# soedinglab/spacedust

Measured on AMD Instinct MI355X. Metric: clustersearch throughput (genome-pairs/s; SW GCUPS alongside), higher is better.
Workload: dtype int16

## Files before the change

### spacedust_amd/csrc/hip/sd_sw.hip

```cpp
#include "sd_common.h"
#include <unistd.h>


#include <algorithm>
#include <cmath>
#include <cstring>
#include <memory>
#include <omp.h>
#include <numeric>

#include "../host/sd_host.h"
#include "sd_sw_pk.h"

namespace {

using sdpk::SwTask;

template <int RT>
__global__ void __launch_bounds__(64)
sw_score_kernel(const SwTask *__restrict__ tasks, uint32_t nTasks, const uint8_t *__restrict__ qRes,
                const int8_t *__restrict__ qBias, const uint8_t *__restrict__ tRes, const int8_t *__restrict__ mat,
                int go, int ge, int32_t *__restrict__ out, uint2 *__restrict__ boundary,
                const uint32_t *__restrict__ order ,
                const int8_t *__restrict__ qProf ) {
// ... 611 lines not shown
            int x = ii - band;
            x = x > 0 ? x : 0;
            x = jj - x;
            ok = ok && x >= 0 && x < width_d;
            bool same = false;
            if (ok) {
                const int byte = dirs[(size_t) 16 * ii + (x >> 1)];
                const int code = (x & 1) ? (byte >> 4) : (byte & 15);
                ok = (code & 12) == 0;
                same = sq[ii] == st[jj];
            }
            const uint32_t okMask = (uint32_t) (__ballot(ok) >> sh);
            const uint32_t sameMask = (uint32_t) (__ballot(same) >> sh);
            const int run = okMask == 0xFFFFFFFFu ? 32 : __builtin_ctz(~okMask);
            const uint32_t runMask = run == 32 ? 0xFFFFFFFFu : ((1u << run) - 1u);
            if (l < run) o[-1 - l] = 'M';
            ids += __builtin_popcount(sameMask & runMask);
            i -= run;
            j -= run;
            o -= run;
            len += run;
        }
        if (going && (i > 0 || j > 0)) {
            if (i < 0 || j < 0) bad = true;
            int x = i - band;
            x = x > 0 ? x : 0;
            x = j - x;
            if (x < 0 || x >= width_d) bad = true;
            if (!bad) {
                const int byte = dirs[(size_t) 16 * i + (x >> 1)];
                const int code = (x & 1) ? (byte >> 4) : (byte & 15);
                int dcode;
                const int dE = (code & 1) ? 3 : 2, dF = (code & 2) ? 5 : 4;
                if (state == 0) dcode = dE;
                else if (state == 1) dcode = dF;
                else dcode = (code & 4) ? dE : ((code & 8) ? dF : 1);
                char c;
                switch (dcode) {
                    case 1: ids += (sq[i] == st[j]); --i; --j; state = 2; c = 'M'; break;
                    case 2: --i; state = 0; c = 'I'; break;
                    case 3: --i; state = 2; c = 'I'; break;
                    case 4: --j; state = 1; c = 'D'; break;
                    default: --j; state = 2; c = 'D'; break;
                }
                --o;
                if (l == 0) *o = c;
                len++;
            }
        }
        going = going && !bad && (i > 0 || j > 0);
    }
    if (!have || !reached || l != 0) return;
    if (bad || i != 0 || j != 0) {
        res[2 * id] = -1;
        return;
    }
    ids += (sq[0] == st[0]);
    *--o = 'M';
    len++;
    res[2 * id] = len;
    res[2 * id + 1] = ids;
}

template <int RT, int LW, bool MULTI, bool WIDE, bool SHARED>
void launchScorePk(sd_ctx *ctx, const SwTask *dTasks, const uint32_t *dOrder, uint32_t n, const sd_seqset *q,
                   const sd_seqset *t, const int8_t *dMat, int go, int ge, int32_t *dOut, uint2 *dBound) {
    if (n == 0) return;
    constexpr uint32_t perWave = 2 * (64 / LW);
    dim3 grid((n + perWave - 1) / perWave), block(64);
    hipLaunchKernelGGL((sdpk::sw_score_pk_kernel<RT, LW, MULTI, WIDE, SHARED>), grid, block, 0, ctx->stream, dTasks, n, q->dRes, q->dBias,
                       t->dRes, dMat, go, ge, dOut, dBound, dOrder, (const int8_t *) q->dProf);
}

template <int RT, bool SHARED>
void launchScorePkAligned(sd_ctx *ctx, const SwTask *dTasks, const uint32_t *dOrder, uint32_t n, const sd_seqset *q, const sd_seqset *t,
                          const int8_t *dMat, int go, int ge, int32_t *dOut) {
    if (n == 0) return;
    constexpr uint32_t perWave = 4;
    dim3 grid((n + perWave - 1) / perWave), block(64);
    hipLaunchKernelGGL((sdpk::sw_score_pk_aligned_kernel<RT, SHARED>), grid, block, 0, ctx->stream, dTasks, n, q->dRes, q->dBias, t->dRes,
                       dMat, go, ge, dOut, dOrder, (const int8_t *) q->dProf);
}

int rtClass(int n) {
    if (n <= 128) return 4;
    if (n <= 256) return 8;
    if (n <= 512) return 16;
    return 32;
}

template <int RT>
void launchScore(sd_ctx *ctx, const SwTask *dTasks, uint32_t n, const sd_seqset *q, const sd_seqset *t,
                 const int8_t *dMat, int go, int ge, int32_t *dOut, uint2 *dBound) {
    if (n == 0) return;
    dim3 grid((n + 1) / 2), block(64);
    hipLaunchKernelGGL(sw_score_kernel<RT>, grid, block, 0, ctx->stream, dTasks, n, q->dRes, q->dBias, t->dRes, dMat,
                       go, ge, dOut, dBound, (const uint32_t *) nullptr, (const int8_t *) q->dProf);
}

template <int RT>
void launchScoreIdx(sd_ctx *ctx, const SwTask *dTasks, const uint32_t *dOrder, uint32_t n, const sd_seqset *q,
                    const sd_seqset *t, const int8_t *dMat, int go, int ge, int32_t *dOut, uint2 *dBound) {
    if (n == 0) return;
    dim3 grid((n + 1) / 2), block(64);
    hipLaunchKernelGGL(sw_score_kernel<RT>, grid, block, 0, ctx->stream, dTasks, n, q->dRes, q->dBias, t->dRes, dMat,
                       go, ge, dOut, dBound, dOrder, (const int8_t *) q->dProf);
}

int runScoreTasks(sd_ctx *ctx, std::vector<SwTask> &tasks, const sd_seqset *q, const sd_seqset *t, const int8_t *dMat,
                  int go, int ge, std::vector<int32_t> &hOut, uint32_t nSlots, uint64_t *cells, const char *tag = "a") {
    hOut.assign((size_t) nSlots * 3, 0);
    if (tasks.empty()) return SD_OK;
    HostScope hsAll(ctx, "score.total");
    const size_t n = tasks.size();
    constexpr int NB = 4 * 1024;
    auto keyOf = [](const SwTask &t) {
        const int c = rtClass(t.n);
        const int ci = c == 4 ? 0 : (c == 8 ? 1 : (c == 16 ? 2 : 3));
        return (uint32_t) ci * 1024u + (uint32_t) (1023 - std::min(t.tL >> 4, 1023));
    };
    SwTask *sorted = nullptr;
    SD_HIP(ctx, pinGet(ctx, (std::string("sw.tasks.") + tag).c_str(), n, &sorted));
    uint64_t boundTotal = 0, cellSum = 0;
    size_t classBegin[5] = {0, 0, 0, 0, 0};
    {
        int T = 1;
#pragma omp parallel
        {
#pragma omp single
            T = omp_get_num_threads();
        }
        T = std::max(1, std::min(T, 64));
        std::vector<uint32_t> hist((size_t) T * NB, 0);
#pragma omp parallel num_threads(T) reduction(+ : cellSum)
        {
            const int th = omp_get_thread_num();
            const size_t lo = n * th / T, hi = n * (th + 1) / T;
            uint32_t *hh = &hist[(size_t) th * NB];
            for (size_t i = lo; i < hi; i++) {
                hh[keyOf(tasks[i])]++;
                cellSum += (uint64_t) tasks[i].n * (uint64_t) tasks[i].tL;
            }
        }
        uint64_t run = 0;
        for (int bkt = 0; bkt < NB; bkt++) {
            if ((bkt & 1023) == 0) classBegin[bkt >> 10] = run;
            for (int th = 0; th < T; th++) {
                const uint32_t c = hist[(size_t) th * NB + bkt];
                hist[(size_t) th * NB + bkt] = (uint32_t) run;
                run += c;
            }
        }
        classBegin[4] = run;
#pragma omp parallel num_threads(T)
        {
            const int th = omp_get_thread_num();
            const size_t lo = n * th / T, hi = n * (th + 1) / T;
            uint32_t *hh = &hist[(size_t) th * NB];
            for (size_t i = lo; i < hi; i++) sorted[hh[keyOf(tasks[i])]++] = tasks[i];
        }
    }
    *cells += cellSum;
    for (size_t i = classBegin[3]; i < classBegin[4]; i++) {
        if (sorted[i].n > 1024) {
            sorted[i].boundOff = boundTotal;
            boundTotal += (uint64_t) sorted[i].tL;
        }
    }
    SwTask *dTasks = nullptr;
    int32_t *dOut = nullptr;
    uint2 *dBound = nullptr;
    int32_t *hPin = nullptr;
    SD_HIP(ctx, wsGet(ctx, "sw.tasks", n, &dTasks));
    SD_HIP(ctx, wsGet(ctx, "sw.out", (size_t) nSlots * 3, &dOut));
    SD_HIP(ctx, wsGet(ctx, "sw.bound", std::max<uint64_t>(boundTotal, 1), &dBound));
    SD_HIP(ctx, pinGet(ctx, "sw.hout", (size_t) nSlots * 3, &hPin));
    SD_HIP(ctx, hipMemcpyAsync(dTasks, sorted, n * sizeof(SwTask), hipMemcpyHostToDevice, ctx->stream));
    SD_HIP(ctx, hipMemsetAsync(dOut, 0, (size_t) nSlots * 3 * sizeof(int32_t), ctx->stream));
    static const int classes[4] = {4, 8, 16, 32};
    for (int ci = 0; ci < 4; ci++) {
        const size_t begin = classBegin[ci], end = classBegin[ci + 1];
        if (end == begin) continue;
        const uint32_t cnt = (uint32_t) (end - begin);
        {
            ProfScope ps(ctx, "sw_score");
            switch (classes[ci]) {
                case 4: launchScore<4>(ctx, dTasks + begin, cnt, q, t, dMat, go, ge, dOut, dBound); break;
                case 8: launchScore<8>(ctx, dTasks + begin, cnt, q, t, dMat, go, ge, dOut, dBound); break;
                case 16: launchScore<16>(ctx, dTasks + begin, cnt, q, t, dMat, go, ge, dOut, dBound); break;
                default: launchScore<32>(ctx, dTasks + begin, cnt, q, t, dMat, go, ge, dOut, dBound); break;
            }
        }
        SD_HIP(ctx, hipGetLastError());
    }
    SD_HIP(ctx, hipMemcpyAsync(hPin, dOut, (size_t) nSlots * 3 * sizeof(int32_t), hipMemcpyDeviceToHost, ctx->stream));
    SD_HIP(ctx, sdStreamSync(ctx));
    memcpy(hOut.data(), hPin, (size_t) nSlots * 3 * sizeof(int32_t));
    return SD_OK;
}


constexpr uint32_t N_NARROW_CLASSES = 24;
constexpr uint32_t FIRST_NARROW_MULTI = 21;
constexpr uint32_t N_PK_CLASSES = 14;
constexpr uint32_t FIRST_MULTI_PK = 11;
constexpr uint32_t FIRST_WIDE_CLASS = N_NARROW_CLASSES;
constexpr uint32_t FIRST_INT32_CLASS = FIRST_WIDE_CLASS + N_PK_CLASSES;
constexpr uint32_t N_SCORE_CLASSES = FIRST_INT32_CLASS + 4;
static_assert(N_SCORE_CLASSES < 63, "class boundaries are found by one 64-lane wavefront; six class bits in the pair key");
enum ScoreKernel { SCORE_PK = 0, SCORE_PK_WIDE = 1, SCORE_INT32 = 2 };
constexpr uint32_t KEY_INVALID = N_SCORE_CLASSES * 1024u;
__host__ __device__ __forceinline__ bool scoreClassIsMulti(uint32_t ci) {
    return (ci >= FIRST_NARROW_MULTI && ci < FIRST_WIDE_CLASS) || (ci >= FIRST_WIDE_CLASS + FIRST_MULTI_PK && ci < FIRST_INT32_CLASS);
}
__device__ __forceinline__ uint32_t scoreKey(int n, int tL, int kernel, int wideRowLimit = 800) {
    int ci;
    if (kernel == SCORE_PK_WIDE && min(n, tL) > wideRowLimit) kernel = SCORE_INT32;
    if (kernel == SCORE_INT32 || tL > 65535) {
        ci = FIRST_INT32_CLASS + (n <= 128 ? 0 : (n <= 256 ? 1 : (n <= 512 ? 2 : 3)));
    } else if (kernel == SCORE_PK_WIDE) {
        if (n <= 192) ci = n <= 128 ? 0 : 1;
        else if (n <= 384) ci = 2 + (n - 193) / 32;
        else if (n <= 768) ci = n <= 512 ? 8 : (n <= 640 ? 9 : 10);
        else ci = min((int) FIRST_MULTI_PK + (n + 511) / 512 - 2, 13);
        ci += FIRST_WIDE_CLASS;
    } else {
        if (n <= 128) ci = 0;
        else if (n <= 768) ci = (n + 31) / 32 - 4;
        else ci = min((int) FIRST_NARROW_MULTI + (n + 511) / 512 - 2, (int) FIRST_WIDE_CLASS - 1);
    }
    return (uint32_t) ci * 1024u + (uint32_t) (1023 - min(tL >> 4, 1023));
}

struct DevGateParams {
    int go, ge, matMin, swMode, covMode, wideRowLimit;
    float covThr;
    double evalThr;
    double lambda, K, aI, bI, alphaI, betaI, aJ, bJ, alphaJ, betaJ, sigma, tau, viThr, vjThr, cThr, dbResidues;
};

__device__ double devEvalue(const DevGateParams &e, double y_, double qLen) {
    const double m_ = e.dbResidues, n_ = qLen;
    const double const_val = 0.3989422804014327;
    double tmp = e.aI * y_ + e.bI;
    double m_li_y = m_ - tmp;
    double vi_y = fmax(e.viThr, e.alphaI * y_ + e.betaI);
    double sqrt_vi_y = sqrt(vi_y);
    double m_F = sqrt_vi_y == 0.0 ? 1e100 : m_li_y / sqrt_vi_y;
    double P_m_F = 0.5 * erfc(-sqrt(0.5) * m_F);
    double E_m_F = -const_val * exp(-0.5 * m_F * m_F);
    double p1 = m_li_y * P_m_F - sqrt_vi_y * E_m_F;
    tmp = e.aJ * y_ + e.bJ;
    double n_lj_y = n_ - tmp;
    double vj_y = fmax(e.vjThr, e.alphaJ * y_ + e.betaJ);
    double sqrt_vj_y = sqrt(vj_y);
    double n_F = sqrt_vj_y == 0.0 ? 1e100 : n_lj_y / sqrt_vj_y;
    double P_n_F = 0.5 * erfc(-sqrt(0.5) * n_F);
    double E_n_F = -const_val * exp(-0.5 * n_F * n_F);
    double p2 = n_lj_y * P_n_F - sqrt_vj_y * E_n_F;
    double c_y = fmax(e.cThr, e.sigma * y_ + e.tau);
    double area = p1 * p2 + c_y * (P_m_F * P_n_F);
    return e.K * exp(-e.lambda * y_) * area;
}

__device__ __forceinline__ float devCov(unsigned int startPos, unsigned int endPos, unsigned int len) {
    return (min(len, max(startPos, endPos)) - min(startPos, endPos) + 1) / (float) len;
}
__device__ __forceinline__ bool devHasCoverage(float covThr, int covMode, float qCov, float tCov) {
    switch (covMode) {
        case 0: return (qCov >= covThr) && (tCov >= covThr);
        case 2: return qCov >= covThr;
        case 1: return tCov >= covThr;
        default: return true;
    }
}

__global__ void __launch_bounds__(256)
k_pre_word(uint32_t nPairs, const uint32_t *__restrict__ pairQ, const uint32_t *__restrict__ pairT, const uint16_t *__restrict__ pairDiag,
           const uint32_t *__restrict__ fwdKeys, const uint64_t *__restrict__ qOff, const uint64_t *__restrict__ tOff,
           const uint8_t *__restrict__ qRes, const int8_t *__restrict__ qBias, const uint8_t *__restrict__ tRes, const int8_t *__restrict__ mat,
           const int8_t *__restrict__ qProf, const int32_t *__restrict__ minBias, int matMin, uint8_t *__restrict__ preWord,
           uint32_t *__restrict__ pass1Keys) {
    __shared__ int8_t smat[441];
    for (int x = threadIdx.x; x < 441; x += blockDim.x) smat[x] = mat[x];
    __syncthreads();
    const uint32_t i = blockIdx.x * blockDim.x + threadIdx.x;
    if (i >= nPairs) return;
    uint8_t pw = 0;
    const uint32_t key = fwdKeys[i];
    if (key != KEY_INVALID) {
        const uint64_t qo = qOff[pairQ[i]], to = tOff[pairT[i]];
        const int qL = (int) (qOff[pairQ[i] + 1] - qo), tL = (int) (tOff[pairT[i] + 1] - to);
        if (qL < 32768 && tL < 32768 && pairDiag[i] != 0x8000) {
            const int d = (int) (int16_t) pairDiag[i];
            int q0 = d >= 0 ? d : 0, t0 = d >= 0 ? 0 : -d;
            const int n = min(qL - q0, tL - t0);
            const int need = 255 - (abs(matMin) + abs(minBias[pairQ[i]]));
            int run = 0, best = 0;
            for (int x = 0; x < n && best < need; x++) {
                const int qr = qRes[qo + q0 + x], tr = tRes[to + t0 + x];
                run += qProf ? (int) qProf[(qo + q0 + x) * 21 + tr] : (int) smat[tr * 21 + qr] + (int) qBias[qo + q0 + x];
                run = run < 0 ? 0 : run;
                best = run > best ? run : best;
            }
            pw = best >= need ? 1 : 0;
        }
    }
// ... 357 lines not shown
    if (!keep) {
        res[i].btLen = 0;
        btLen[i] = 0;
    }
}

__global__ void __launch_bounds__(256)
k_accept(uint32_t nPairs, const sd_sw_result *__restrict__ res, const uint8_t *__restrict__ ident, uint8_t *__restrict__ acc) {
    const uint32_t i = blockIdx.x * blockDim.x + threadIdx.x;
    if (i >= nPairs) return;
    const sd_sw_result &r = res[i];
    acc[i] = (ident[i] || (r.btLen > 0 && r.qStart >= 0 && r.tStart >= 0)) ? 1 : 0;
}
__global__ void __launch_bounds__(256)
k_accept_compact(uint32_t nPairs, const sd_sw_result *__restrict__ res, const uint8_t *__restrict__ acc,
                 const uint64_t *__restrict__ pos, sd_sw_result *__restrict__ outRes, uint32_t *__restrict__ outIdx) {
    const uint32_t i = blockIdx.x * blockDim.x + threadIdx.x;
    if (i >= nPairs || !acc[i]) return;
    outRes[pos[i]] = res[i];
    outIdx[pos[i]] = i;
}
#include "sd_scan_sort.h"

template <typename T>
int devExclusiveScan(sd_ctx *ctx, const T *in, uint64_t *out, size_t n) {
    uint64_t *tmp = nullptr;
    SD_HIP(ctx, wsGet(ctx, "al.scantmp", sdScanTmpBytes(n) / sizeof(uint64_t) + 32, &tmp));
    SD_HIP(ctx, (sdScanLaunch<T, ScanSum64, false, uint64_t>(ctx->stream, in, out, n, tmp)));
    return SD_OK;
}
int devInclusiveMax(sd_ctx *ctx, const uint32_t *in, uint32_t *out, size_t n) {
    uint32_t *tmp = nullptr;
    SD_HIP(ctx, wsGet(ctx, "al.scantmp32", sdScanTmpBytes(n) / sizeof(uint32_t) + 32, &tmp));
    SD_HIP(ctx, (sdScanLaunch<uint32_t, ScanMax32, true, uint32_t>(ctx->stream, in, out, n, tmp)));
    return SD_OK;
}

int devSortPairs(sd_ctx *ctx, const uint32_t *kIn, uint32_t *kOut, const uint32_t *vIn, uint32_t *vOut, size_t n, int endBit) {
    if (n == 0) return SD_OK;
    uint32_t *kTmp = nullptr, *vTmp = nullptr, *cnt = nullptr;
    SD_HIP(ctx, wsGet(ctx, "al.sortK", n, &kTmp));
    SD_HIP(ctx, wsGet(ctx, "al.sortV", n, &vTmp));
    SD_HIP(ctx, wsGet(ctx, "al.sortCounts", sdRadixSortCountsBytes() / sizeof(uint32_t), &cnt));
    SD_HIP(ctx, sdRadixSortPairs(ctx->stream, kIn, vIn, kOut, vOut, kTmp, vTmp, (uint32_t) n, 0, endBit, cnt));
    return SD_OK;
}

__global__ void __launch_bounds__(256)
k_bound_need(uint32_t nPairs, const SwTask *__restrict__ tasks, const uint32_t *__restrict__ keys, uint64_t *__restrict__ need) {
    const uint32_t i = blockIdx.x * blockDim.x + threadIdx.x;
    if (i >= nPairs) return;
    uint64_t v = 0;
    if (keys[i] != KEY_INVALID) {
        const uint32_t ci = keys[i] >> 10;
        if (scoreClassIsMulti(ci)) v = 2ull * (uint64_t) tasks[i].tL;
        else if (ci == N_SCORE_CLASSES - 1 && tasks[i].n > 1024) v = (uint64_t) tasks[i].tL;
    }
    need[i] = v;
}
__global__ void __launch_bounds__(256)
k_bound_apply(uint32_t nPairs, SwTask *__restrict__ tasks, const uint64_t *__restrict__ off) {
    const uint32_t i = blockIdx.x * blockDim.x + threadIdx.x;
    if (i >= nPairs) return;
    tasks[i].boundOff = off[i];
}

constexpr uint32_t PAIR_NONE = 0xFFFFFFFFu;
constexpr int PAIR_QUERY_BITS = 17;
__global__ void __launch_bounds__(256)
k_pair_keys(uint32_t n, const uint32_t *__restrict__ keys, const uint32_t *__restrict__ pairQ, uint32_t *__restrict__ key2) {
    const uint32_t i = blockIdx.x * blockDim.x + threadIdx.x;
    if (i >= n) return;
    const uint32_t k = keys[i];
    key2[i] = k == KEY_INVALID ? 0xFFFFFFFFu : ((k >> 10) << 26) | (pairQ[i] << 9) | ((k & 1023u) >> 1);
}
__global__ void __launch_bounds__(256)
k_pair_heads(uint32_t n, const uint32_t *__restrict__ keyS, uint32_t *__restrict__ headPos) {
    const uint32_t p = blockIdx.x * blockDim.x + threadIdx.x;
    if (p >= n) return;
    const bool head = p == 0 || (keyS[p] >> 9) != (keyS[p - 1] >> 9);
    headPos[p] = head ? p : 0u;
}
__global__ void __launch_bounds__(256)
k_pair_leaders(uint32_t n, const uint32_t *__restrict__ keyS, const uint32_t *__restrict__ runStart, uint8_t *__restrict__ leader) {
    const uint32_t p = blockIdx.x * blockDim.x + threadIdx.x;
    if (p > n) return;
    uint8_t v = 0;
    if (p < n && (keyS[p] >> 26) < FIRST_INT32_CLASS) {
        const uint32_t o = p - runStart[p];
        v = (o & 1u) == 0 ? 1 : 0;
        const bool lastOfRun = p + 1 >= n || (keyS[p + 1] >> 9) != (keyS[p] >> 9);
        const uint32_t pairs = (o + 1 + 1) / 2;
        if (lastOfRun) v += (uint8_t) (pairs & 1u);
    }
    leader[p] = v;
}
__global__ void __launch_bounds__(256)
k_pair_emit(uint32_t n, const uint32_t *__restrict__ keyS, const uint32_t *__restrict__ vals, const uint32_t *__restrict__ runStartOf,
            const uint64_t *__restrict__ pairIdx, uint32_t *__restrict__ order2) {
    const uint32_t p = blockIdx.x * blockDim.x + threadIdx.x;
    if (p >= n || (keyS[p] >> 26) >= FIRST_INT32_CLASS || ((p - runStartOf[p]) & 1u)) return;
    const uint64_t w = pairIdx[p];
    order2[2 * w] = vals[p];
    const bool mate = p + 1 < n && (keyS[p + 1] >> 9) == (keyS[p] >> 9);
    order2[2 * w + 1] = mate ? vals[p + 1] : PAIR_NONE;
}
__global__ void k_pair_bounds(const uint32_t *__restrict__ keyS, uint32_t n, const uint64_t *__restrict__ pairIdx,
                              uint32_t *__restrict__ b, int nb) {
    const int c = threadIdx.x;
    if (c >= nb) return;
    const uint32_t want = (uint32_t) c << 26;
    uint32_t lo = 0, hi = n;
    while (lo < hi) {
        const uint32_t mid = (lo + hi) >> 1;
        if (keyS[mid] < want) lo = mid + 1;
        else hi = mid;
    }
    b[c] = (uint32_t) pairIdx[lo];
}

int devRunScore(sd_ctx *ctx, uint32_t nPairs, const uint32_t *dKeys, const uint32_t *dVals, uint32_t *dKeysSorted,
                uint32_t *dOrder, uint32_t *dBounds, SwTask *dTasks, uint64_t *dScanA, uint64_t *dScanB,
                const sd_seqset *q, const sd_seqset *t, const int8_t *dMat, int go, int ge, int32_t *dOut,
                uint32_t *nValid, const uint32_t *dPairQ ) {
    const unsigned grid = (nPairs + 255) / 256;
    int rc = SD_OK;
    uint32_t *dOrder2 = nullptr, *dPairBounds = nullptr;
    if (dPairQ) {
        uint32_t *dKey2 = nullptr, *dVals2 = nullptr, *dHead = nullptr, *dRunStart = nullptr;
        uint64_t *dPairIdx = nullptr;
        uint8_t *dLeader = nullptr;
        SD_HIP(ctx, wsGet(ctx, "sp.key2", (size_t) nPairs, &dKey2));
        SD_HIP(ctx, wsGet(ctx, "sp.vals2", (size_t) nPairs, &dVals2));
        SD_HIP(ctx, wsGet(ctx, "sp.head", (size_t) nPairs, &dHead));
        SD_HIP(ctx, wsGet(ctx, "sp.runstart", (size_t) nPairs, &dRunStart));
        SD_HIP(ctx, wsGet(ctx, "sp.leader", (size_t) nPairs + 1, &dLeader));
        SD_HIP(ctx, wsGet(ctx, "sp.pairidx", (size_t) nPairs + 1, &dPairIdx));
        const size_t order2Cap = (size_t) 4 * nPairs + 8;
        SD_HIP(ctx, wsGet(ctx, "sp.order2", order2Cap, &dOrder2));
        SD_HIP(ctx, hipMemsetAsync(dOrder2, 0xFF, order2Cap * sizeof(uint32_t), ctx->stream));
        SD_HIP(ctx, wsGet(ctx, "sp.bounds", 64, &dPairBounds));
        hipLaunchKernelGGL(k_pair_keys, dim3(grid), dim3(256), 0, ctx->stream, nPairs, dKeys, dPairQ, dKey2);
        rc = devSortPairs(ctx, dKey2, dKeysSorted, dVals, dVals2, nPairs, 32);
        if (rc != SD_OK) return rc;
        dOrder = dVals2;
        hipLaunchKernelGGL(k_pair_heads, dim3(grid), dim3(256), 0, ctx->stream, nPairs, dKeysSorted, dHead);
        rc = devInclusiveMax(ctx, dHead, dRunStart, nPairs);
        if (rc != SD_OK) return rc;
        hipLaunchKernelGGL(k_pair_leaders, dim3((nPairs + 256) / 256), dim3(256), 0, ctx->stream, nPairs, dKeysSorted, dRunStart, dLeader);
        rc = devExclusiveScan(ctx, (const uint8_t *) dLeader, dPairIdx, (size_t) nPairs + 1);
        if (rc != SD_OK) return rc;
        hipLaunchKernelGGL(k_pair_emit, dim3(grid), dim3(256), 0, ctx->stream, nPairs, dKeysSorted, dVals2, dRunStart, dPairIdx, dOrder2);
        hipLaunchKernelGGL(k_pair_bounds, dim3(1), dim3(64), 0, ctx->stream, dKeysSorted, nPairs, dPairIdx, dPairBounds,
                           (int) FIRST_INT32_CLASS + 1);
        hipLaunchKernelGGL(k_bounds, dim3(1), dim3(64), 0, ctx->stream, dKeysSorted, nPairs, 1u << 26, dBounds, (int) N_SCORE_CLASSES + 1);
    } else {
        rc = devSortPairs(ctx, dKeys, dKeysSorted, dVals, dOrder, nPairs, 16);
        if (rc != SD_OK) return rc;
        hipLaunchKernelGGL(k_bounds, dim3(1), dim3(64), 0, ctx->stream, dKeysSorted, nPairs, 1024u, dBounds, (int) N_SCORE_CLASSES + 1);
    }
    hipLaunchKernelGGL(k_bound_need, dim3(grid), dim3(256), 0, ctx->stream, nPairs, dTasks, dKeys, dScanA);
    SD_HIP(ctx, hipMemsetAsync(dScanA + nPairs, 0, sizeof(uint64_t), ctx->stream));
    rc = devExclusiveScan(ctx, dScanA, dScanB, (size_t) nPairs + 1);
    if (rc != SD_OK) return rc;
    hipLaunchKernelGGL(k_bound_apply, dim3(grid), dim3(256), 0, ctx->stream, nPairs, dTasks, dScanB);
    uint32_t hb[N_SCORE_CLASSES + 1], hpb[FIRST_INT32_CLASS + 1];
    uint64_t boundTotal = 0;
    if (dPairQ) SD_HIP(ctx, sdD2H(ctx, hpb, dPairBounds, sizeof(hpb)));
    SD_HIP(ctx, sdD2H(ctx, hb, dBounds, sizeof(hb)));
    SD_HIP(ctx, sdD2H(ctx, &boundTotal, dScanB + nPairs, sizeof(uint64_t)));
    SD_HIP(ctx, sdStreamSync(ctx));
    *nValid = hb[N_SCORE_CLASSES];
    uint2 *dBound = nullptr;
    SD_HIP(ctx, wsGet(ctx, "sw.bound", std::max<uint64_t>(boundTotal, 1), &dBound));
    for (uint32_t ci = 0; ci < N_SCORE_CLASSES; ci++) {
        const uint32_t begin = hb[ci], cnt = hb[ci + 1] - hb[ci];
        if (cnt == 0) continue;
        static const char *const pkNames[N_PK_CLASSES] = {"rt4x32", "rt6x32", "rt7x32", "rt8x32", "rt9x32", "rt10x32", "rt11x32", "rt12x32",
                                                          "rt8x64", "rt10x64", "rt12x64", "rt8x64s2", "rt8x64s3", "rt8x64sN"};
        static const char *const i32Names[4] = {"sw_score.rt4", "sw_score.rt8", "sw_score.rt16", "sw_score.rt32"};
        const bool shared = dPairQ != nullptr && ci < FIRST_INT32_CLASS;
        const int alignedRT = (ci >= 1 && ci < FIRST_NARROW_MULTI) ? (int) ci + 4 : 0;
        const bool aligned = alignedRT > 0 && (alignedRT <= 12 || shared);
        int generalIdx = 0;
        if (ci >= FIRST_NARROW_MULTI && ci < FIRST_WIDE_CLASS) generalIdx = (int) FIRST_MULTI_PK + (int) (ci - FIRST_NARROW_MULTI);
        else if (alignedRT) generalIdx = alignedRT <= 6 ? 1 : (alignedRT <= 12 ? alignedRT - 5 : (alignedRT <= 16 ? 8 : (alignedRT <= 20 ? 9 : 10)));
        char name[48];
        if (aligned) snprintf(name, sizeof(name), "sw_score_pk.a_seg%d", alignedRT);
        else if (ci < FIRST_WIDE_CLASS) snprintf(name, sizeof(name), "sw_score_pk.%s", pkNames[generalIdx]);
        else if (ci < FIRST_INT32_CLASS) snprintf(name, sizeof(name), "sw_score_pk.w_%s", pkNames[ci - FIRST_WIDE_CLASS]);
        else snprintf(name, sizeof(name), "%s", i32Names[ci - FIRST_INT32_CLASS]);
        ProfScope ps(ctx, name);
        const uint32_t *ord = dOrder + begin;
        uint32_t nOrd = cnt;
        if (shared) {
            ord = dOrder2 + 2 * (size_t) hpb[ci];
            nOrd = 2 * (hpb[ci + 1] - hpb[ci]);
        }
#define SD_PK(RT, LW, MULTI, WIDE)                                                                                          \
    do {                                                                                                                   \
        if (shared) launchScorePk<RT, LW, MULTI, WIDE, true>(ctx, dTasks, ord, nOrd, q, t, dMat, go, ge, dOut, dBound);     \
        else launchScorePk<RT, LW, MULTI, WIDE, false>(ctx, dTasks, ord, nOrd, q, t, dMat, go, ge, dOut, dBound);           \
    } while (0)
#define SD_PKA(RT)                                                                                       \
    case RT:                                                                                             \
        if (shared) launchScorePkAligned<RT, true>(ctx, dTasks, ord, nOrd, q, t, dMat, go, ge, dOut);    \
        else launchScorePkAligned<RT, false>(ctx, dTasks, ord, nOrd, q, t, dMat, go, ge, dOut);          \
        break;
#define SD_PK_CLASS(WIDE, IDX)                                                \
        switch (IDX) {                                                        \
            case 0: SD_PK(4, 32, false, WIDE); break;                         \
            case 1: SD_PK(6, 32, false, WIDE); break;                         \
            case 2: SD_PK(7, 32, false, WIDE); break;                         \
            case 3: SD_PK(8, 32, false, WIDE); break;                         \
            case 4: SD_PK(9, 32, false, WIDE); break;                         \
            case 5: SD_PK(10, 32, false, WIDE); break;                        \
            case 6: SD_PK(11, 32, false, WIDE); break;                        \
            case 7: SD_PK(12, 32, false, WIDE); break;                        \
            case 8: SD_PK(8, 64, false, WIDE); break;                         \
            case 9: SD_PK(10, 64, false, WIDE); break;                        \
            case 10: SD_PK(12, 64, false, WIDE); break;                       \
            default: SD_PK(8, 64, true, WIDE); break;                         \
        }
        if (aligned) {
            switch (alignedRT) {
                SD_PKA(5) SD_PKA(6) SD_PKA(7) SD_PKA(8) SD_PKA(9) SD_PKA(10) SD_PKA(11) SD_PKA(12) SD_PKA(13) SD_PKA(14)
                SD_PKA(15) SD_PKA(16) SD_PKA(17) SD_PKA(18) SD_PKA(19) SD_PKA(20) SD_PKA(21) SD_PKA(22) SD_PKA(23) SD_PKA(24)
                default: break;
            }
        } else if (ci < FIRST_WIDE_CLASS) {
            SD_PK_CLASS(false, generalIdx)
        } else if (ci < FIRST_INT32_CLASS) {
            SD_PK_CLASS(true, (int) (ci - FIRST_WIDE_CLASS))
        } else {
            switch (ci - FIRST_INT32_CLASS) {
                case 0: launchScoreIdx<4>(ctx, dTasks, ord, cnt, q, t, dMat, go, ge, dOut, dBound); break;
                case 1: launchScoreIdx<8>(ctx, dTasks, ord, cnt, q, t, dMat, go, ge, dOut, dBound); break;
                case 2: launchScoreIdx<16>(ctx, dTasks, ord, cnt, q, t, dMat, go, ge, dOut, dBound); break;
                default: launchScoreIdx<32>(ctx, dTasks, ord, cnt, q, t, dMat, go, ge, dOut, dBound); break;
            }
        }
#undef SD_PKA
#undef SD_PK_CLASS
#undef SD_PK
    }
    SD_HIP(ctx, hipGetLastError());
    return SD_OK;
}

__global__ void __launch_bounds__(256)
k_cells(uint32_t nPairs, const SwTask *__restrict__ tasks, const uint32_t *__restrict__ keys, unsigned long long *__restrict__ acc) {
    const uint32_t i = blockIdx.x * blockDim.x + threadIdx.x;
    unsigned long long c = 0;
    if (i < nPairs && keys[i] != KEY_INVALID) c = (unsigned long long) tasks[i].n * (unsigned long long) tasks[i].tL;
#pragma unroll
    for (int off = 32; off >= 1; off >>= 1) c += __shfl_xor(c, off, 64);
    if ((threadIdx.x & 63) == 0 && c) atomicAdd(acc, c);
}

}

int sdFail(sd_ctx *ctx, int code, const char *fmt, ...) {
    char buf[1024];
    va_list ap;
    va_start(ap, fmt);
    vsnprintf(buf, sizeof(buf), fmt, ap);
    va_end(ap);
    if (ctx) ctx->lastError = buf;
    else fprintf(stderr, "spacedust_gpu: %s\n", buf);
    return code;
}

extern "C" {

int sd_ctx_create(int device, sd_ctx **out) { return sd_ctx_create_prio(device, 0, out); }

int sd_ctx_create_prio(int device, int priority, sd_ctx **out) { return sd_ctx_create_masked(device, priority, 0, out); }

int sd_ctx_create_masked(int device, int priority, int reserveCUs, sd_ctx **out) {
    if (out == nullptr) return SD_EINVAL;
    *out = nullptr;
    int count = 0;
    hipError_t e = hipGetDeviceCount(&count);
    if (e != hipSuccess || count <= 0) {
        fprintf(stderr, "spacedust_gpu: no HIP device visible (%s); this library has no CPU fallback\n",
                e != hipSuccess ? hipGetErrorString(e) : "device count 0");
        return SD_ENODEVICE;
    }
    if (device < 0 || device >= count) return SD_EINVAL;
    if (hipSetDevice(device) != hipSuccess) return SD_ENODEVICE;
    sd_ctx *c = new sd_ctx();
    c->device = device;
    int least = 0, greatest = 0;
    (void) hipDeviceGetStreamPriorityRange(&least, &greatest);
    const int prio = priority < 0 ? greatest : (priority > 0 ? least : (least + greatest) / 2);
    hipError_t se = hipSuccess;
    (void) hipGetDeviceProperties(&c->prop, device);
    const int nCU = c->prop.multiProcessorCount;
    if (reserveCUs > 0 && nCU > 0 && reserveCUs < nCU) {
        std::vector<uint32_t> mask((size_t) (nCU + 31) / 32, 0u);
        for (int b = 0; b < nCU - reserveCUs; b++) mask[(size_t) b / 32] |= 1u << (b % 32);
        se = hipExtStreamCreateWithCUMask(&c->stream, (uint32_t) mask.size(), mask.data());
    } else {
        se = hipStreamCreateWithPriority(&c->stream, hipStreamNonBlocking, prio);
    }
    if (se != hipSuccess) {
        delete c;
        return SD_EHIP;
    }
    const char *syncMode = getenv("SD_SYNC");
    const bool spin = syncMode && strcmp(syncMode, "spin") == 0;
    (void) hipEventCreate(&c->evStart);
    (void) hipEventCreate(&c->evStop);
    if (!spin) (void) hipEventCreateWithFlags(&c->evSync, hipEventDisableTiming);
    (void) hipGetDeviceProperties(&c->prop, device);
    *out = c;
    return SD_OK;
}

void sd_ctx_destroy(sd_ctx *ctx) {
    if (!ctx) return;
    (void) hipSetDevice(ctx->device);
    if (ctx->evStart) (void) hipEventDestroy(ctx->evStart);
    if (ctx->evStop) (void) hipEventDestroy(ctx->evStop);
// ... 1106 lines not shown
```

### spacedust_amd/csrc/hip/sd_sw_pk.h

```cpp
#ifndef SD_SW_PK_H
#define SD_SW_PK_H

#include <hip/hip_runtime.h>
#include <cstdint>

namespace sdpk {

struct SwTask {
    uint64_t qOff;
    uint64_t tOff;
    int32_t n;
    int32_t tL;
    int32_t qStep;
    int32_t tStep;
    int32_t segLen;
    uint32_t slot;
    uint64_t boundOff;
};

typedef short s16x2 __attribute__((ext_vector_type(2)));
typedef unsigned short u16x2 __attribute__((ext_vector_type(2)));

__device__ __forceinline__ uint32_t pkMax(uint32_t a, uint32_t b) {
    return __builtin_bit_cast(uint32_t, __builtin_elementwise_max(__builtin_bit_cast(s16x2, a), __builtin_bit_cast(s16x2, b)));
// ... 495 lines not shown
            chunk = chunkNext;
            chunkNext = loadChunk(k + 1 + LW);
        }
        Tn = dppShr1(Tc);
        Tn = writeLane<0>(readLane(chunk, i1), Tn);
        Tn = writeLane<32>(readLane(chunk, 32 + i1), Tn);
        {
            const uint32_t aA = addWord0(baseA, Tn), aB = addWord1(baseB, Tn);
#pragma unroll
            for (int w = 0; w < WORDS; w++) {
                pan[w] = ldsWord(aA, w);
                pbn[w] = ldsWord(aB, w);
            }
        }
        uint32_t inG = dppShr1(outG), inFf = dppShr1(outFf);
        inG = writeLane<32>(0, inG);
        inFf = writeLane<32>(0, inFf);
        uint32_t h[RTP];
#pragma unroll
        for (int w = 0; w < WORDS; w++) {
            const uint32_t d0 = (w == 0) ? prevInG : H[4 * w - 1];
            addProfile4(pac[w], pbc[w], d0, H[4 * w], H[4 * w + 1], H[4 * w + 2], h[4 * w], h[4 * w + 1], h[4 * w + 2], h[4 * w + 3]);
        }
        prevInG = inG;
        uint32_t Fl = 0, Ff = inFf, cm = 0;
#pragma unroll
        for (int r = 0; r < RT; r++) {
            uint32_t hpre = pkMax(h[r], E[r]);
            if (r != 0) hpre = pkMax(hpre, Fl);
            const uint32_t g = pkMax(hpre, Ff);
            const uint32_t open = pkSubSat(hpre, goP);
            E[r] = pkMax(pkSubSat(E[r], geP), open);
            if (r == 0) Fl = open;
            else if (r + 1 != RT) Fl = pkMax(pkSubSat(Fl, geP), open);
            Ff = pkMax(pkSubSat(Ff, geP), open);
            H[r] = g;
            const uint32_t code = pkRowCode(g, 31 - r);
            cm = r == 0 ? code : pkMax(cm, code);
        }
        outG = H[RT - 1];
        outFf = Ff;
        const uint32_t t = bestcm | 0x001F001Fu;
        const uint32_t m = pkAshr15(pkSub(t, cm));
        const uint32_t kk = (uint32_t) k | ((uint32_t) k << 16);
        bestcm = bfiAsm(m, cm, bestcm);
        bestcol = bfiAsm(m, kk, bestcol);
    };
    uint32_t T2, pa2[WORDS], pb2[WORDS];
#pragma unroll 1
    for (int k = 0; k < steps; k += 2) {
        columnStep(k, T, pa, pb, T2, pa2, pb2);
        columnStep(k + 1, T2, pa2, pb2, T, pa, pb);
    }
    unsigned long long keyA = 0, keyB = 0;
    {
        const uint32_t vA = (bestcm & 0xFFFFu) >> 5, vB = bestcm >> 21;
        const uint32_t rowA = (uint32_t) (q0 + 31 - (int) (bestcm & 31u)), rowB = (uint32_t) (q0 + 31 - (int) ((bestcm >> 16) & 31u));
        const uint32_t colA = (bestcol & 0xFFFFu) - (uint32_t) l, colB = (bestcol >> 16) - (uint32_t) l;
        if (vA > 0) keyA = ((unsigned long long) vA << 40) | ((unsigned long long) (0xFFFFFu - colA) << 20) | (unsigned long long) (0xFFFFFu - rowA);
        if (vB > 0) keyB = ((unsigned long long) vB << 40) | ((unsigned long long) (0xFFFFFu - colB) << 20) | (unsigned long long) (0xFFFFFu - rowB);
    }
#pragma unroll
    for (int off = LW / 2; off >= 1; off >>= 1) {
        const unsigned long long oa = __shfl_xor(keyA, off, LW), ob = __shfl_xor(keyB, off, LW);
        keyA = oa > keyA ? oa : keyA;
        keyB = ob > keyB ? ob : keyB;
    }
    if (l == 0) {
        if (haveA) {
            const int v = (int) (keyA >> 40);
            out[3 * A.slot + 0] = v;
            out[3 * A.slot + 1] = v == 0 ? -1 : 0xFFFFF - (int) ((keyA >> 20) & 0xFFFFF);
            out[3 * A.slot + 2] = v == 0 ? A.n - 1 : 0xFFFFF - (int) (keyA & 0xFFFFF);
        }
        if (haveB) {
            const int v = (int) (keyB >> 40);
            out[3 * B.slot + 0] = v;
            out[3 * B.slot + 1] = v == 0 ? -1 : 0xFFFFF - (int) ((keyB >> 20) & 0xFFFFF);
            out[3 * B.slot + 2] = v == 0 ? B.n - 1 : 0xFFFFF - (int) (keyB & 0xFFFFF);
        }
    }
}

}
#endif
```

Measured before the change: 2640.

## Add word-packed 16-lane SW kernel for wide mid-length classes with finer bucketing

```diff
diff --git a/spacedust_amd/csrc/hip/sd_sw.hip b/spacedust_amd/csrc/hip/sd_sw.hip
--- a/spacedust_amd/csrc/hip/sd_sw.hip
+++ b/spacedust_amd/csrc/hip/sd_sw.hip
@@ -717,6 +717,16 @@
                        dMat, go, ge, dOut, dOrder, (const int8_t *) q->dProf);
 }
 
+template <int RT, bool SHARED>
+void launchScorePkWord(sd_ctx *ctx, const SwTask *dTasks, const uint32_t *dOrder, uint32_t n, const sd_seqset *q, const sd_seqset *t,
+                       const int8_t *dMat, int go, int ge, int32_t *dOut) {
+    if (n == 0) return;
+    constexpr uint32_t perWave = 8;
+    dim3 grid((n + perWave - 1) / perWave), block(64);
+    hipLaunchKernelGGL((sdpk::sw_score_pk_word_kernel<RT, SHARED>), grid, block, 0, ctx->stream, dTasks, n, q->dRes, q->dBias, t->dRes,
+                       dMat, go, ge, dOut, dOrder, (const int8_t *) q->dProf);
+}
+
 int rtClass(int n) {
     if (n <= 128) return 4;
     if (n <= 256) return 8;
@@ -839,14 +849,17 @@
 constexpr uint32_t FIRST_NARROW_MULTI = 21;
 constexpr uint32_t N_PK_CLASSES = 14;
 constexpr uint32_t FIRST_MULTI_PK = 11;
+constexpr uint32_t N_WIDE_CLASSES = 23;
+constexpr uint32_t FIRST_WORD_SEG = 9, LAST_WORD_SEG = 24;
+constexpr uint32_t FIRST_WIDE_MULTI = 20;
 constexpr uint32_t FIRST_WIDE_CLASS = N_NARROW_CLASSES;
-constexpr uint32_t FIRST_INT32_CLASS = FIRST_WIDE_CLASS + N_PK_CLASSES;
+constexpr uint32_t FIRST_INT32_CLASS = FIRST_WIDE_CLASS + N_WIDE_CLASSES;
 constexpr uint32_t N_SCORE_CLASSES = FIRST_INT32_CLASS + 4;
 static_assert(N_SCORE_CLASSES < 63, "class boundaries are found by one 64-lane wavefront; six class bits in the pair key");
 enum ScoreKernel { SCORE_PK = 0, SCORE_PK_WIDE = 1, SCORE_INT32 = 2 };
 constexpr uint32_t KEY_INVALID = N_SCORE_CLASSES * 1024u;
 __host__ __device__ __forceinline__ bool scoreClassIsMulti(uint32_t ci) {
-    return (ci >= FIRST_NARROW_MULTI && ci < FIRST_WIDE_CLASS) || (ci >= FIRST_WIDE_CLASS + FIRST_MULTI_PK && ci < FIRST_INT32_CLASS);
+    return (ci >= FIRST_NARROW_MULTI && ci < FIRST_WIDE_CLASS) || (ci >= FIRST_WIDE_CLASS + FIRST_WIDE_MULTI && ci < FIRST_INT32_CLASS);
 }
 __device__ __forceinline__ uint32_t scoreKey(int n, int tL, int kernel, int wideRowLimit = 800) {
     int ci;
@@ -854,10 +867,10 @@
     if (kernel == SCORE_INT32 || tL > 65535) {
         ci = FIRST_INT32_CLASS + (n <= 128 ? 0 : (n <= 256 ? 1 : (n <= 512 ? 2 : 3)));
     } else if (kernel == SCORE_PK_WIDE) {
-        if (n <= 192) ci = n <= 128 ? 0 : 1;
-        else if (n <= 384) ci = 2 + (n - 193) / 32;
-        else if (n <= 768) ci = n <= 512 ? 8 : (n <= 640 ? 9 : 10);
-        else ci = min((int) FIRST_MULTI_PK + (n + 511) / 512 - 2, 13);
+        if (n <= 128) ci = 0;
+        else if (n <= 384) ci = (n + 15) / 16 - 8;
+        else if (n <= 768) ci = n <= 512 ? 17 : (n <= 640 ? 18 : 19);
+        else ci = min((int) FIRST_WIDE_MULTI + (n + 511) / 512 - 2, (int) N_WIDE_CLASSES - 1);
         ci += FIRST_WIDE_CLASS;
     } else {
         if (n <= 128) ci = 0;
@@ -1381,7 +1394,8 @@
     headPos[p] = head ? p : 0u;
 }
 __global__ void __launch_bounds__(256)
-k_pair_leaders(uint32_t n, const uint32_t *__restrict__ keyS, const uint32_t *__restrict__ runStart, uint8_t *__restrict__ leader) {
+k_pair_leaders(uint32_t n, const uint32_t *__restrict__ keyS, const uint32_t *__restrict__ runStart, uint8_t *__restrict__ leader,
+               int wordAligned) {
     const uint32_t p = blockIdx.x * blockDim.x + threadIdx.x;
     if (p > n) return;
     uint8_t v = 0;
@@ -1390,7 +1404,9 @@
         v = (o & 1u) == 0 ? 1 : 0;
         const bool lastOfRun = p + 1 >= n || (keyS[p + 1] >> 9) != (keyS[p] >> 9);
         const uint32_t pairs = (o + 1 + 1) / 2;
-        if (lastOfRun) v += (uint8_t) (pairs & 1u);
+        const uint32_t ci = keyS[p] >> 26;
+        const bool four = wordAligned && ci > FIRST_WIDE_CLASS && ci <= FIRST_WIDE_CLASS + (LAST_WORD_SEG - FIRST_WORD_SEG + 1);
+        if (lastOfRun) v += (uint8_t) (four ? (4u - (pairs & 3u)) & 3u : pairs & 1u);
     }
     leader[p] = v;
 }
@@ -1424,6 +1440,7 @@
                 uint32_t *nValid, const uint32_t *dPairQ ) {
     const unsigned grid = (nPairs + 255) / 256;
     int rc = SD_OK;
+    const bool wordAligned = !(getenv("SD_SW_WORD_ALIGNED") && atoi(getenv("SD_SW_WORD_ALIGNED")) == 0);
     uint32_t *dOrder2 = nullptr, *dPairBounds = nullptr;
     if (dPairQ) {
         uint32_t *dKey2 = nullptr, *dVals2 = nullptr, *dHead = nullptr, *dRunStart = nullptr;
@@ -1435,7 +1452,7 @@
         SD_HIP(ctx, wsGet(ctx, "sp.runstart", (size_t) nPairs, &dRunStart));
         SD_HIP(ctx, wsGet(ctx, "sp.leader", (size_t) nPairs + 1, &dLeader));
         SD_HIP(ctx, wsGet(ctx, "sp.pairidx", (size_t) nPairs + 1, &dPairIdx));
-        const size_t order2Cap = (size_t) 4 * nPairs + 8;
+        const size_t order2Cap = (size_t) 8 * nPairs + 8;
         SD_HIP(ctx, wsGet(ctx, "sp.order2", order2Cap, &dOrder2));
         SD_HIP(ctx, hipMemsetAsync(dOrder2, 0xFF, order2Cap * sizeof(uint32_t), ctx->stream));
         SD_HIP(ctx, wsGet(ctx, "sp.bounds", 64, &dPairBounds));
@@ -1446,7 +1463,8 @@
         hipLaunchKernelGGL(k_pair_heads, dim3(grid), dim3(256), 0, ctx->stream, nPairs, dKeysSorted, dHead);
         rc = devInclusiveMax(ctx, dHead, dRunStart, nPairs);
         if (rc != SD_OK) return rc;
-        hipLaunchKernelGGL(k_pair_leaders, dim3((nPairs + 256) / 256), dim3(256), 0, ctx->stream, nPairs, dKeysSorted, dRunStart, dLeader);
+        hipLaunchKernelGGL(k_pair_leaders, dim3((nPairs + 256) / 256), dim3(256), 0, ctx->stream, nPairs, dKeysSorted, dRunStart, dLeader,
+                           wordAligned ? 1 : 0);
         rc = devExclusiveScan(ctx, (const uint8_t *) dLeader, dPairIdx, (size_t) nPairs + 1);
         if (rc != SD_OK) return rc;
         hipLaunchKernelGGL(k_pair_emit, dim3(grid), dim3(256), 0, ctx->stream, nPairs, dKeysSorted, dVals2, dRunStart, dPairIdx, dOrder2);
@@ -1484,10 +1502,16 @@
         int generalIdx = 0;
         if (ci >= FIRST_NARROW_MULTI && ci < FIRST_WIDE_CLASS) generalIdx = (int) FIRST_MULTI_PK + (int) (ci - FIRST_NARROW_MULTI);
         else if (alignedRT) generalIdx = alignedRT <= 6 ? 1 : (alignedRT <= 12 ? alignedRT - 5 : (alignedRT <= 16 ? 8 : (alignedRT <= 20 ? 9 : 10)));
+        const uint32_t wi = ci >= FIRST_WIDE_CLASS && ci < FIRST_INT32_CLASS ? ci - FIRST_WIDE_CLASS : 0;
+        const int wordRT = (wi >= 1 && wi < FIRST_WIDE_MULTI - 3) ? (int) (wi + FIRST_WORD_SEG - 1) : 0;
+        const bool wordKernel = wordAligned && wordRT > 0 && (wordRT <= 12 || shared);
+        if (wordRT) generalIdx = wordRT <= 12 ? 1 : 2 + (wordRT - 13) / 2;
+        else if (wi >= FIRST_WIDE_MULTI - 3) generalIdx = 8 + (int) (wi - (FIRST_WIDE_MULTI - 3));
         char name[48];
-        if (aligned) snprintf(name, sizeof(name), "sw_score_pk.a_seg%d", alignedRT);
+        if (wordKernel) snprintf(name, sizeof(name), "sw_score_pk.w_seg%d", wordRT);
+        else if (aligned) snprintf(name, sizeof(name), "sw_score_pk.a_seg%d", alignedRT);
         else if (ci < FIRST_WIDE_CLASS) snprintf(name, sizeof(name), "sw_score_pk.%s", pkNames[generalIdx]);
-        else if (ci < FIRST_INT32_CLASS) snprintf(name, sizeof(name), "sw_score_pk.w_%s", pkNames[ci - FIRST_WIDE_CLASS]);
+        else if (ci < FIRST_INT32_CLASS) snprintf(name, sizeof(name), "sw_score_pk.w_%s", pkNames[generalIdx]);
         else snprintf(name, sizeof(name), "%s", i32Names[ci - FIRST_INT32_CLASS]);
         ProfScope ps(ctx, name);
         const uint32_t *ord = dOrder + begin;
@@ -1521,7 +1545,18 @@
             case 10: SD_PK(12, 64, false, WIDE); break;                       \
             default: SD_PK(8, 64, true, WIDE); break;                         \
         }
-        if (aligned) {
+#define SD_PKW(RT)                                                                                    \
+    case RT:                                                                                          \
+        if (shared) launchScorePkWord<RT, true>(ctx, dTasks, ord, nOrd, q, t, dMat, go, ge, dOut);    \
+        else launchScorePkWord<RT, false>(ctx, dTasks, ord, nOrd, q, t, dMat, go, ge, dOut);          \
+        break;
+        if (wordKernel) {
+            switch (wordRT) {
+                SD_PKW(9) SD_PKW(10) SD_PKW(11) SD_PKW(12) SD_PKW(13) SD_PKW(14) SD_PKW(15) SD_PKW(16) SD_PKW(17) SD_PKW(18) SD_PKW(19)
+                SD_PKW(20) SD_PKW(21) SD_PKW(22) SD_PKW(23) SD_PKW(24)
+                default: break;
+            }
+        } else if (aligned) {
             switch (alignedRT) {
                 SD_PKA(5) SD_PKA(6) SD_PKA(7) SD_PKA(8) SD_PKA(9) SD_PKA(10) SD_PKA(11) SD_PKA(12) SD_PKA(13) SD_PKA(14)
                 SD_PKA(15) SD_PKA(16) SD_PKA(17) SD_PKA(18) SD_PKA(19) SD_PKA(20) SD_PKA(21) SD_PKA(22) SD_PKA(23) SD_PKA(24)
@@ -1530,7 +1565,7 @@
         } else if (ci < FIRST_WIDE_CLASS) {
             SD_PK_CLASS(false, generalIdx)
         } else if (ci < FIRST_INT32_CLASS) {
-            SD_PK_CLASS(true, (int) (ci - FIRST_WIDE_CLASS))
+            SD_PK_CLASS(true, generalIdx)
         } else {
             switch (ci - FIRST_INT32_CLASS) {
                 case 0: launchScoreIdx<4>(ctx, dTasks, ord, cnt, q, t, dMat, go, ge, dOut, dBound); break;
@@ -1539,6 +1574,7 @@
                 default: launchScoreIdx<32>(ctx, dTasks, ord, cnt, q, t, dMat, go, ge, dOut, dBound); break;
             }
         }
+#undef SD_PKW
 #undef SD_PKA
 #undef SD_PK_CLASS
 #undef SD_PK
diff --git a/spacedust_amd/csrc/hip/sd_sw_pk.h b/spacedust_amd/csrc/hip/sd_sw_pk.h
--- a/spacedust_amd/csrc/hip/sd_sw_pk.h
+++ b/spacedust_amd/csrc/hip/sd_sw_pk.h
@@ -601,5 +601,231 @@
     }
 }
 
+__device__ __forceinline__ uint32_t dppRowShr1(uint32_t fill, uint32_t v) {
+    return (uint32_t) __builtin_amdgcn_update_dpp((int) fill, (int) v, 0x111 , 0xf, 0xf, false);
+}
+__device__ __forceinline__ uint32_t dppRowShl1(uint32_t v) {
+    return (uint32_t) __builtin_amdgcn_update_dpp((int) v, (int) v, 0x101 , 0xf, 0xf, false);
+}
+
+template <int RT, bool SHARED>
+__global__ void __launch_bounds__(64)
+sw_score_pk_word_kernel(const SwTask *__restrict__ tasks, uint32_t nTasks, const uint8_t *__restrict__ qRes,
+                        const int8_t *__restrict__ qBias, const uint8_t *__restrict__ tRes, const int8_t *__restrict__ mat,
+                        int go, int ge, int32_t *__restrict__ out, const uint32_t *__restrict__ order,
+                        const int8_t *__restrict__ qProf) {
+    constexpr int LW = 16;
+    constexpr int WORDS = (RT + 3) / 4;
+    constexpr int RTP = 4 * WORDS;
+    constexpr int PSTRIDE = LW * WORDS;
+    constexpr int NGRP = 64 / LW;
+    constexpr int NT = 2 * NGRP;
+    constexpr uint32_t ROWB = PSTRIDE * 4;
+    static_assert(RT <= 32, "the row code has five bits");
+    static_assert(22 * ROWB < 65536, "row offsets travel in 16 bits");
+    __shared__ uint32_t prof[SHARED ? 1 : NT][22][PSTRIDE];
+    __shared__ int8_t smat[441];
+    for (int i = threadIdx.x; i < 441; i += 64) smat[i] = mat[i];
+    __syncthreads();
+    const int lane = threadIdx.x & 63;
+    const int grp = lane / LW, l = lane % LW;
+    auto taskId = [&](uint32_t x) -> uint32_t {
+        const uint32_t id = blockIdx.x * NT + x;
+        return id < nTasks ? (order ? order[id] : id) : 0xFFFFFFFFu;
+    };
+    auto loadTask = [&](uint32_t tid) -> SwTask {
+        SwTask T;
+        if (tid != 0xFFFFFFFFu) {
+            T = tasks[tid];
+        } else {
+            T.n = 0; T.tL = 0; T.qOff = 0; T.tOff = 0; T.qStep = 1; T.tStep = 1; T.segLen = 1; T.slot = 0; T.boundOff = 0;
+        }
+        return T;
+    };
+    const SwTask A = loadTask(taskId(2 * grp));
+    SwTask B = loadTask(taskId(2 * grp + 1));
+    const bool haveA = A.n > 0, haveB = B.n > 0;
+    if (SHARED && !haveB) {
+        B = A;
+        B.tL = 0;
+    }
+    int maxN = 0, maxTL = 0;
+#pragma unroll
+    for (int x = 0; x < NT; x++) {
+        const uint32_t tid = taskId(x);
+        if (tid != 0xFFFFFFFFu) {
+            maxN = max(maxN, tasks[tid].n);
+            maxTL = max(maxTL, tasks[tid].tL);
+        }
+    }
+    const int steps = (maxN > 0 && maxTL > 0) ? maxTL + LW - 1 : 0;
+    const uint32_t goP = (uint32_t) go | ((uint32_t) go << 16), geP = (uint32_t) ge | ((uint32_t) ge << 16);
+    const int q0 = l * RT;
+#pragma unroll
+    for (int x = 0; x < (SHARED ? 1 : 2); x++) {
+        const SwTask T = SHARED ? loadTask(taskId(0)) : (x ? B : A);
+        uint32_t *pw = &prof[SHARED ? 0 : 2 * grp + x][0][0] + l * WORDS;
+#pragma unroll
+        for (int w = 0; w < WORDS; w++) {
+            int res[4], cb[4];
+            int64_t pidx[4];
+            bool valid[4];
+#pragma unroll
+            for (int b = 0; b < 4; b++) {
+                const int qi = q0 + 4 * w + b;
+                valid[b] = (4 * w + b < RT) && qi < T.n;
+                res[b] = 20;
+                cb[b] = 0;
+                pidx[b] = 0;
+                if (valid[b]) {
+                    const int64_t idx = (int64_t) T.qOff + (int64_t) qi * T.qStep;
+                    res[b] = qRes[idx];
+                    cb[b] = qBias[idx];
+                    pidx[b] = idx * 21;
+                }
+            }
+            const int aFirst = SHARED ? grp : 0, aStep = SHARED ? NGRP : 1;
+            if (qProf) {
+                for (int a = aFirst; a < 21; a += aStep) {
+                    uint32_t word = 0;
+#pragma unroll
+                    for (int b = 0; b < 4; b++) {
+                        const int v = valid[b] ? (int) qProf[pidx[b] + a] : -64;
+                        word |= (uint32_t) (uint8_t) (int8_t) v << (8 * b);
+                    }
+                    pw[a * PSTRIDE + w] = word;
+                }
+            } else {
+                for (int a = aFirst; a < 21; a += aStep) {
+                    uint32_t word = 0;
+#pragma unroll
+                    for (int b = 0; b < 4; b++) {
+                        const int v = valid[b] ? (int) smat[a * 21 + res[b]] + cb[b] : -64;
+                        word |= (uint32_t) (uint8_t) (int8_t) v << (8 * b);
+                    }
+                    pw[a * PSTRIDE + w] = word;
+                }
+            }
+            pw[PK_NEUTRAL * PSTRIDE + w] = 0xC0C0C0C0u;
+        }
+    }
+    __syncthreads();
+    typedef __attribute__((address_space(3))) uint32_t lds_u32;
+    const uint32_t baseA = (uint32_t) (size_t) (lds_u32 *) (&prof[SHARED ? 0 : 2 * grp][0][0] + l * WORDS);
+    const uint32_t baseB = SHARED ? baseA : (uint32_t) (size_t) (lds_u32 *) (&prof[SHARED ? 0 : 2 * grp + 1][0][0] + l * WORDS);
+    auto ldsWord = [](uint32_t addr, int w) -> uint32_t { return *((const lds_u32 *) (size_t) addr + w); };
+
+    uint32_t H[RTP], E[RTP];
+#pragma unroll
+    for (int r = 0; r < RTP; r++) {
+        H[r] = 0;
+        E[r] = 0;
+    }
+    uint32_t outG = 0, outFf = 0, prevInG = 0;
+    uint32_t bestA = 0, bestB = 0, bcolA = 0, bcolB = 0;
+    constexpr uint32_t NEUT = (uint32_t) PK_NEUTRAL * ROWB;
+    auto loadChunk = [&](int c0) -> uint32_t {
+        const int col = c0 + l;
+        uint32_t a = PK_NEUTRAL, b = PK_NEUTRAL;
+        if (col < A.tL) a = tRes[(int64_t) A.tOff + (int64_t) col * A.tStep];
+        if (col < B.tL) b = tRes[(int64_t) B.tOff + (int64_t) col * B.tStep];
+        return (a * ROWB) | ((b * ROWB) << 16);
+    };
+    uint32_t chunk = loadChunk(0);
+    uint32_t chunkNext = loadChunk(LW);
+    uint32_t T = l == 0 ? chunk : (NEUT | (NEUT << 16));
+    uint32_t pa[WORDS], pb[WORDS];
+    {
+        const uint32_t aA = addWord0(baseA, T), aB = addWord1(baseB, T);
+#pragma unroll
+        for (int w = 0; w < WORDS; w++) {
+            pa[w] = ldsWord(aA, w);
+            pb[w] = ldsWord(aB, w);
+        }
+    }
+    auto columnStep = [&](const int k, const uint32_t &Tc, const uint32_t (&pac)[WORDS], const uint32_t (&pbc)[WORDS], uint32_t &Tn,
+                          uint32_t (&pan)[WORDS], uint32_t (&pbn)[WORDS]) {
+        if (((k + 1) & (LW - 1)) == 0) {
+            chunk = chunkNext;
+            chunkNext = loadChunk(k + 1 + LW);
+        } else {
+            chunk = dppRowShl1(chunk);
+        }
+        Tn = dppRowShr1(chunk, Tc);
+        {
+            const uint32_t aA = addWord0(baseA, Tn), aB = addWord1(baseB, Tn);
+#pragma unroll
+            for (int w = 0; w < WORDS; w++) {
+                pan[w] = ldsWord(aA, w);
+                pbn[w] = ldsWord(aB, w);
+            }
+        }
+        const uint32_t inG = dppRowShr1(0, outG), inFf = dppRowShr1(0, outFf);
+        uint32_t h[RTP];
+#pragma unroll
+        for (int w = 0; w < WORDS; w++) {
+            const uint32_t d0 = (w == 0) ? prevInG : H[4 * w - 1];
+            addProfile4(pac[w], pbc[w], d0, H[4 * w], H[4 * w + 1], H[4 * w + 2], h[4 * w], h[4 * w + 1], h[4 * w + 2], h[4 * w + 3]);
+        }
+        prevInG = inG;
+        uint32_t Fl = 0, Ff = inFf, cmA = 0, cmB = 0;
+#pragma unroll
+        for (int r = 0; r < RT; r++) {
+            uint32_t hpre = pkMax(h[r], E[r]);
+            if (r != 0) hpre = pkMax(hpre, Fl);
+            const uint32_t g = pkMax(hpre, Ff);
+            const uint32_t open = pkSubSat(hpre, goP);
+            E[r] = pkMax(pkSubSat(E[r], geP), open);
+            if (r == 0) Fl = open;
+            else if (r + 1 != RT) Fl = pkMax(pkSubSat(Fl, geP), open);
+            Ff = pkMax(pkSubSat(Ff, geP), open);
+            H[r] = g;
+            cmA = max(cmA, (g << 16) | (uint32_t) (31 - r));
+            cmB = max(cmB, (g & 0xFFFF0000u) | (uint32_t) (31 - r));
+        }
+        outG = H[RT - 1];
+        outFf = Ff;
+        const bool upA = cmA > (bestA | 0xFFFFu), upB = cmB > (bestB | 0xFFFFu);
+        bestA = upA ? cmA : bestA;
+        bcolA = upA ? (uint32_t) k : bcolA;
+        bestB = upB ? cmB : bestB;
+        bcolB = upB ? (uint32_t) k : bcolB;
+    };
+    uint32_t T2, pa2[WORDS], pb2[WORDS];
+#pragma unroll 1
+    for (int k = 0; k < steps; k += 2) {
+        columnStep(k, T, pa, pb, T2, pa2, pb2);
+        columnStep(k + 1, T2, pa2, pb2, T, pa, pb);
+    }
+    unsigned long long keyA = 0, keyB = 0;
+    {
+        const uint32_t vA = bestA >> 16, vB = bestB >> 16;
+        const uint32_t rowA = (uint32_t) (q0 + 31 - (int) (bestA & 31u)), rowB = (uint32_t) (q0 + 31 - (int) (bestB & 31u));
+        const uint32_t colA = bcolA - (uint32_t) l, colB = bcolB - (uint32_t) l;
+        if (vA > 0) keyA = ((unsigned long long) vA << 40) | ((unsigned long long) (0xFFFFFu - colA) << 20) | (unsigned long long) (0xFFFFFu - rowA);
+        if (vB > 0) keyB = ((unsigned long long) vB << 40) | ((unsigned long long) (0xFFFFFu - colB) << 20) | (unsigned long long) (0xFFFFFu - rowB);
+    }
+#pragma unroll
+    for (int off = LW / 2; off >= 1; off >>= 1) {
+        const unsigned long long oa = __shfl_xor(keyA, off, LW), ob = __shfl_xor(keyB, off, LW);
+        keyA = oa > keyA ? oa : keyA;
+        keyB = ob > keyB ? ob : keyB;
+    }
+    if (l == 0) {
+        if (haveA) {
+            const int v = (int) (keyA >> 40);
+            out[3 * A.slot + 0] = v;
+            out[3 * A.slot + 1] = v == 0 ? -1 : 0xFFFFF - (int) ((keyA >> 20) & 0xFFFFF);
+            out[3 * A.slot + 2] = v == 0 ? A.n - 1 : 0xFFFFF - (int) (keyA & 0xFFFFF);
+        }
+        if (haveB) {
+            const int v = (int) (keyB >> 40);
+            out[3 * B.slot + 0] = v;
+            out[3 * B.slot + 1] = v == 0 ? -1 : 0xFFFFF - (int) ((keyB >> 20) & 0xFFFFF);
+            out[3 * B.slot + 2] = v == 0 ? B.n - 1 : 0xFFFFF - (int) (keyB & 0xFFFFF);
+        }
+    }
+}
+
 }
 #endif
```

New measurement: 2663, median of 4. Within noise of the previous version (+0.9%).
